# xuanjiangliu/robotic-discovery-platform

Measured on AMD Instinct MI355X. Metric: U-Net train imgs/sec at 256×256 (1/2/4/8 GPU); e2e frames/sec + p50 latency, higher is better.
Workload: dtype bf16; 1 GPU; model=UNet(3,1) bilinear decoder, 17.26M params, global_batch=64, per_gpu_batch=64, image_size=256, parallelism=dp1, impl=native, optimizer=Adam(lr=1e-4), loss=bce, sync_bn=False, hipgraph=False

## Files before the change

csrc/bindings.cpp:

```cpp
#include <torch/extension.h>
#include <c10/hip/HIPGuard.h>
#include <c10/hip/HIPStream.h>
#include <hip/hip_runtime.h>
#include <dlfcn.h>
#include <link.h>
#include <chrono>
#include <cmath>
#include <climits>
#include <cstdlib>
#include <cstring>
#include <functional>
#include <memory>
#include <vector>
#include <array>

#include "rdp_api.h"

namespace {

hipStream_t cur_stream() { return c10::hip::getCurrentHIPStream().stream(); }

void note_device(int& dev, const torch::Tensor& t) {
  if (!t.defined() || !t.is_cuda()) return;
  const int d = t.get_device();
// ... 698 lines not shown
  TORCH_CHECK(o.N == a.N && o.H == a.H && o.W == a.W && o.C == a.C, "bn bwd apply shape");
  TORCH_CHECK(RDP_PLAN(rdp_bn_relu_bwd_apply(d.ptr, d.pitch, a.ptr, a.pitch, coef.data_ptr<float>(), coef2.data_ptr<float>(),
                                    o.ptr, o.pitch, a.N * a.H * a.W, a.C, relu, st)) == 0, "bn bwd apply");
}

void maxpool2_fwd(torch::Tensor x, torch::Tensor out) {
  Act a = act(x, "x"), o = act(out, "out");
  TORCH_CHECK(o.N == a.N && o.H == a.H / 2 && o.W == a.W / 2 && o.C == a.C, "maxpool shape");
  TORCH_CHECK(RDP_PLAN(rdp_maxpool2_fwd(a.ptr, a.pitch, o.ptr, o.pitch, a.N, a.H, a.W, a.C, st)) == 0, "maxpool");
}

void maxpool2_bwd(torch::Tensor dp, torch::Tensor x, c10::optional<torch::Tensor> dskip, torch::Tensor dx) {
  Act p = act(dp, "dp"), a = act(x, "x"), o = act(dx, "dx"), s;
  if (dskip) { s = act(*dskip, "dskip"); TORCH_CHECK(s.N == a.N && s.H == a.H && s.W == a.W && s.C == a.C, "dskip shape"); }
  TORCH_CHECK(p.N == a.N && p.H == a.H / 2 && p.W == a.W / 2 && p.C == a.C, "maxpool bwd shape");
  TORCH_CHECK(o.N == a.N && o.H == a.H && o.W == a.W && o.C == a.C, "maxpool bwd dx shape");
  TORCH_CHECK(RDP_PLAN(rdp_maxpool2_bwd(p.ptr, p.pitch, a.ptr, a.pitch, dskip ? s.ptr : nullptr, dskip ? s.pitch : 0, o.ptr,
                               o.pitch, a.N, a.H, a.W, a.C, st)) == 0, "maxpool bwd");
}

void bn_relu_apply_pool(torch::Tensor y, c10::optional<torch::Tensor> out, torch::Tensor pool, torch::Tensor coef) {
  Act a = act(y, "y"), o, p = act(pool, "pool");
  if (out) {
    o = act(*out, "out");
    TORCH_CHECK(a.N == o.N && a.H == o.H && a.W == o.W && a.C == o.C, "bn_relu_apply_pool shape");
  }
  TORCH_CHECK(p.N == a.N && p.H == a.H / 2 && p.W == a.W / 2 && p.C == a.C, "bn_relu_apply_pool pool shape");
  check_f32(coef, "coef");
  TORCH_CHECK(coef.numel() >= 4 * a.C, "coef");
  TORCH_CHECK(RDP_PLAN(rdp_bn_relu_apply_pool(a.ptr, a.pitch, out ? o.ptr : nullptr, out ? o.pitch : 0, p.ptr, p.pitch, coef.data_ptr<float>(), a.N, a.H,
                                     a.W, a.C, st)) == 0, "bn_relu_apply_pool: channels must be 2^k in [8, 2048]");
}

int maxpool2_bwd_bn_reduce(torch::Tensor dp, torch::Tensor x, c10::optional<torch::Tensor> dskip, torch::Tensor dx,
                           torch::Tensor y, torch::Tensor coef, torch::Tensor partial) {
  Act p = act(dp, "dp"), a = act(x, "x"), o = act(dx, "dx"), yy = act(y, "y"), s;
  if (dskip) { s = act(*dskip, "dskip"); TORCH_CHECK(s.N == a.N && s.H == a.H && s.W == a.W && s.C == a.C, "dskip shape"); }
  TORCH_CHECK(p.N == a.N && p.H == a.H / 2 && p.W == a.W / 2 && p.C == a.C, "maxpool bwd shape");
  TORCH_CHECK(o.N == a.N && o.H == a.H && o.W == a.W && o.C == a.C, "maxpool bwd dx shape");
  TORCH_CHECK(yy.N == a.N && yy.H == a.H && yy.W == a.W && yy.C == a.C, "maxpool bwd y shape");
  check_f32(coef, "coef");
  check_f32(partial, "partial");
  TORCH_CHECK(coef.numel() >= 4 * a.C, "coef");
  const int maxb = partial.numel() / (2 * a.C);
  TORCH_CHECK(maxb >= 1, "partial too small");
  const int T = RDP_PLAN(rdp_maxpool2_bwd_bn_reduce(p.ptr, p.pitch, a.ptr, a.pitch, dskip ? s.ptr : nullptr, dskip ? s.pitch : 0,
                                           o.ptr, o.pitch, yy.ptr, yy.pitch, coef.data_ptr<float>(), a.N, a.H, a.W, a.C,
                                           partial.data_ptr<float>(), maxb, st));
  TORCH_CHECK(T > 0, "maxpool2_bwd_bn_reduce: channels must be 2^k in [8, 2048]");
  return T;
}

void upsample2_fwd(torch::Tensor x, torch::Tensor out, int oy, int ox, c10::optional<torch::Tensor> coef) {
  Act a = act(x, "x"), o = act(out, "out");
  TORCH_CHECK(o.N == a.N && o.C == a.C, "upsample shape");
  TORCH_CHECK(2 * a.H + oy <= o.H && 2 * a.W + ox <= o.W && oy >= 0 && ox >= 0, "upsample fwd placement");
  const float* cp = nullptr;
  if (coef && coef->defined()) {
    TORCH_CHECK(coef->is_cuda() && coef->scalar_type() == torch::kFloat32 && coef->numel() >= 4 * a.C, "coef [4C] f32");
    cp = coef->data_ptr<float>();
  }
  TORCH_CHECK(RDP_PLAN(rdp_upsample2_fwd(a.ptr, a.pitch, o.ptr, o.pitch, a.N, a.H, a.W, o.H, o.W, oy, ox, a.C, cp,
                                st)) == 0,
              "upsample fwd: channels must be 2^k in [8, 2048], pitches multiples of 8");
}

int upsample2_bwd(torch::Tensor dout, torch::Tensor dx, int oy, int ox, c10::optional<torch::Tensor> y,
                  c10::optional<torch::Tensor> coef, c10::optional<torch::Tensor> partial) {
  Act d = act(dout, "dout"), o = act(dx, "dx"), yy;
  TORCH_CHECK(o.N == d.N && o.C == d.C, "upsample bwd shape");
  TORCH_CHECK(2 * o.H + oy <= d.H && 2 * o.W + ox <= d.W && oy >= 0 && ox >= 0, "upsample bwd placement");
  const float* cf = nullptr;
  float* pp = nullptr;
  int maxb = 0;
  if (y) {
    TORCH_CHECK(coef && partial, "upsample2_bwd: y needs coef and partial");
    yy = act(*y, "y");
    TORCH_CHECK(yy.N == o.N && yy.H == o.H && yy.W == o.W && yy.C == o.C, "upsample bwd y shape");
    check_f32(*coef, "coef");
    check_f32(*partial, "partial");
    TORCH_CHECK(coef->numel() >= 4 * o.C, "coef");
    maxb = std::min<long>(partial->numel() / (2 * o.C), 4096);
    TORCH_CHECK(maxb >= 1, "partial too small");
// ... 1004 lines not shown
  m.def("plan_pause", &plan_pause);
  m.def("plan_resume", &plan_resume);
  m.def("plan_size", &plan_size);
  m.def("plan_free", &plan_free);
  m.def("conv_fwd", on_device(&conv_fwd), py::arg("x1"), py::arg("x2"), py::arg("w"), py::arg("taps"), py::arg("packed"),
        py::arg("y1"), py::arg("y2"), py::arg("stats"), py::arg("bm_pref"), py::arg("affine"), py::arg("relu"),
        py::arg("ws") = py::none(), py::arg("pool") = py::none(), py::arg("up") = py::none(),
        py::arg("up_oy") = 0, py::arg("up_ox") = 0, py::arg("wfrag") = py::none());
  m.def("conv_ws_elems", [](int N, int H, int W, int C1, int C2, int Cout, int taps, int packed, int bm_pref) {
    return rdp_conv_ws_elems(N, H, W, C1, C2, Cout, taps, packed, bm_pref);
  });
  m.def("conv_stats_rows", &conv_stats_rows);
  m.def("conv_wgrad", on_device(&conv_wgrad), py::arg("x1"), py::arg("x2"), py::arg("dy"), py::arg("taps"),
        py::arg("packed"), py::arg("cin_real"), py::arg("slab"), py::arg("out"), py::arg("accumulate"),
        py::arg("splits"), py::arg("variant"));
  m.def("conv_fwd_bnin", on_device(&conv_fwd_bnin), py::arg("x_pre"), py::arg("w"), py::arg("y"), py::arg("stats"),
        py::arg("in_coef"), py::arg("a_out") = py::none());
  m.def("wgrad_first_bn", on_device(&wgrad_first_bn));
  m.def("wgrad_slab_elems", &wgrad_slab_elems);
  m.def("wgrad_halo_slab_elems", &rdp_conv_wgrad_halo_slab_elems);
  m.def("bn_finalize", on_device(&bn_finalize));
  m.def("bn_eval_coef", on_device(&bn_eval_coef));
  m.def("bn_relu_apply", on_device(&bn_relu_apply));
  m.def("bn_relu_bwd_reduce", on_device(&bn_relu_bwd_reduce));
  m.def("conv_dgrad_bnred", on_device(&conv_dgrad_bnred));
  m.def("conv_dgrad_splitk_bnred", on_device(&conv_dgrad_splitk_bnred), py::arg("dy"), py::arg("w"), py::arg("dx"),
        py::arg("y_bn"), py::arg("coef"), py::arg("partial"), py::arg("ws") = py::none());
  m.def("bn_bwd_finalize", on_device(&bn_bwd_finalize));
  m.def("bn_relu_bwd_apply", on_device(&bn_relu_bwd_apply));
  m.def("maxpool2_fwd", on_device(&maxpool2_fwd));
  m.def("maxpool2_bwd", on_device(&maxpool2_bwd));
  m.def("bn_relu_apply_pool", on_device(&bn_relu_apply_pool));
  m.def("maxpool2_bwd_bn_reduce", on_device(&maxpool2_bwd_bn_reduce));
  m.def("upsample2_fwd", on_device(&upsample2_fwd), py::arg("x"), py::arg("out"), py::arg("oy"), py::arg("ox"),
        py::arg("coef") = py::none());
  m.def("upT_shuffle", on_device(&upT_shuffle));
  m.def("conv_upT_fwd", on_device(&conv_upT_fwd));
  m.def("conv_upT_dgrad", on_device(&conv_upT_dgrad));
  m.def("conv_wgrad_upT", on_device(&conv_wgrad_upT));
  m.def("upT_unshuffle", on_device(&upT_unshuffle));
  m.def("colsum_bf16", on_device(&colsum_bf16));
  m.def("upsample2_bwd", on_device(&upsample2_bwd), py::arg("dout"), py::arg("dx"), py::arg("oy"), py::arg("ox"),
        py::arg("y") = py::none(), py::arg("coef") = py::none(), py::arg("partial") = py::none());
  m.def("head_partial_blocks", &head_partial_blocks);
  m.def("head_fwd", on_device(&head_fwd), py::arg("a"), py::arg("w"), py::arg("b"), py::arg("target"), py::arg("logits"),
        py::arg("partial"), py::arg("sums"), py::arg("loss"), py::arg("dice_w"), py::arg("dice_eps"),
        py::arg("coef") = py::none(), py::arg("gpart") = py::none(), py::arg("bnpart") = py::none(),
        py::arg("gscale") = 1.0);
  m.def("head_grad_finalize", on_device(&head_grad_finalize));
  m.def("head_bwd", on_device(&head_bwd), py::arg("a"), py::arg("w"), py::arg("logits"), py::arg("target"), py::arg("sums"),
        py::arg("da"), py::arg("partial"), py::arg("gw"), py::arg("gb"), py::arg("dice_w"), py::arg("dice_eps"),
        py::arg("gscale"), py::arg("coef") = py::none(), py::arg("bnpart") = py::none());
  m.def("head_bn_bwd_apply", on_device(&head_bn_bwd_apply));
  m.def("head_mask", on_device(&head_mask));
  m.def("headk_partial_blocks", &headk_partial_blocks);
  m.def("headk_fwd", on_device(&headk_fwd), py::arg("a"), py::arg("w"), py::arg("b"), py::arg("labels"),
        py::arg("logits"), py::arg("partial"), py::arg("sums"), py::arg("loss"), py::arg("class_weights") = py::none(),
        py::arg("dice_w") = 0.0, py::arg("dice_eps") = 1.0);
  m.def("headk_bwd", on_device(&headk_bwd), py::arg("a"), py::arg("w"), py::arg("logits"), py::arg("labels"),
        py::arg("sums"), py::arg("da"), py::arg("partial"), py::arg("gw"), py::arg("gb"), py::arg("gscale") = 1.0,
        py::arg("class_weights") = py::none(), py::arg("dice_w") = 0.0, py::arg("dice_eps") = 1.0);
  m.def("headk_mask", on_device(&headk_mask), py::arg("a"), py::arg("w"), py::arg("b"), py::arg("cls"),
        py::arg("mask"));
  m.def("seg_confusion_blocks", &seg_confusion_blocks);
  m.def("seg_confusion_block_pixels", &seg_confusion_block_pixels);
  m.def("seg_confusion", on_device(&seg_confusion), py::arg("logits"), py::arg("target"), py::arg("K"),
// ... 63 lines not shown
```

csrc/pool_up.hip:

```cpp
#include "common.h"
#include "rdp_api.h"
#include <algorithm>

RDP_DEV void unpack8f(const uint4& v, float* f) {
  const uint32_t w[4] = {v.x, v.y, v.z, v.w};
#pragma unroll
  for (int k = 0; k < 4; ++k) {
    f[2 * k] = __uint_as_float(w[k] << 16);
    f[2 * k + 1] = __uint_as_float(w[k] & 0xffff0000u);
  }
}
RDP_DEV uint4 pack8f(const float* f) {
  uint4 v;
  v.x = pack2bf(f[0], f[1]);
  v.y = pack2bf(f[2], f[3]);
  v.z = pack2bf(f[4], f[5]);
  v.w = pack2bf(f[6], f[7]);
  return v;
}

__global__ void maxpool2_fwd_kernel(const u16* __restrict__ x, int xpitch, u16* __restrict__ out, int opitch, int N,
                                    int H, int W, int C) {
  const int Ho = H / 2, Wo = W / 2, CG = C >> 3;
  const long total = (long)N * Ho * Wo * CG;
// ... 103 lines not shown
    for (int q = 0; q < 4; ++q) {
      const int h = 2 * hc + (q >> 1), w = 2 * wc + (q & 1);
      ok[q] = h < H && w < W;
      px[q] = ((long)n * H + h) * W + w;
      if (ok[q]) v[q] = *(const uint4*)(y + px[q] * ypitch + c);
    }
    float av[4][8];
#pragma unroll
    for (int q = 0; q < 4; ++q) {
      if (!ok[q]) continue;
      float f[8];
      unpack8f(v[q], f);
#pragma unroll
      for (int k = 0; k < 8; ++k) f[k] = fmaxf(fmaf(f[k], ss[k], hh[k]), 0.f);
      const uint4 o = pack8f(f);
      if (a) *(uint4*)(a + px[q] * apitch + c) = o;
      unpack8f(o, av[q]);
    }
    if (hc < Ho && wc < Wo) {
      float o[8];
#pragma unroll
      for (int k = 0; k < 8; ++k) {
        float m = av[0][k];
#pragma unroll
        for (int q = 1; q < 4; ++q)
          if (av[q][k] > m || isnan(av[q][k])) m = av[q][k];
        o[k] = m;
      }
      *(uint4*)(pool + (((long)n * Ho + hc) * Wo + wc) * ppitch + c) = pack8f(o);
    }
  }
}

__global__ __launch_bounds__(256) void maxpool2_bwd_bn_reduce_kernel(
    const u16* __restrict__ dp, int dppitch, const u16* __restrict__ dskip,
    int dspitch, u16* __restrict__ dx, int dxpitch, const u16* __restrict__ y, int ypitch,
    const float* __restrict__ coef, int N, int H, int W, int C, float* __restrict__ partial) {
  extern __shared__ __attribute__((aligned(16))) float sred[];
  const int CG = C >> 3, RPB = 256 / CG;
  const int g = threadIdx.x & (CG - 1), r = threadIdx.x / CG;
  const int c = g * 8;
  float mean[8], inv[8], ss[8], hh[8];
  ld8f(coef + c, mean);
  ld8f(coef + C + c, inv);
  ld8f(coef + 2 * C + c, ss);
  ld8f(coef + 3 * C + c, hh);
  float sg[8], sgx[8];
#pragma unroll
  for (int k = 0; k < 8; ++k) { sg[k] = 0.f; sgx[k] = 0.f; }
  const int Ho = H / 2, Wo = W / 2, Hc = (H + 1) / 2, Wc = (W + 1) / 2;
  const int nwin = N * Hc * Wc;
  for (int wi = blockIdx.x * RPB + r; wi < nwin; wi += gridDim.x * RPB) {
    const int wc = wi % Wc, t = wi / Wc;
    const int hc = t % Hc, n = t / Hc;
    const bool pooled = hc < Ho && wc < Wo;
    bool ok[4];
    long px[4];
    uint4 vs[4], vy[4], vd;
#pragma unroll
    for (int q = 0; q < 4; ++q) {
      const int h = 2 * hc + (q >> 1), w = 2 * wc + (q & 1);
      ok[q] = h < H && w < W;
      px[q] = ((long)n * H + h) * W + w;
      if (ok[q]) {
        vy[q] = *(const uint4*)(y + px[q] * ypitch + c);
        vs[q] = dskip ? *(const uint4*)(dskip + px[q] * dspitch + c) : make_uint4(0, 0, 0, 0);
// ... 1 lines not shown
    }
    if (pooled) vd = *(const uint4*)(dp + (((long)n * Ho + hc) * Wo + wc) * dppitch + c);
    int idx[8];
    float d[8];
    if (pooled) {
      float v[4][8];
#pragma unroll
      for (int q = 0; q < 4; ++q) {
        float f[8];
        unpack8f(vy[q], f);
#pragma unroll
        for (int k = 0; k < 8; ++k) f[k] = fmaxf(fmaf(f[k], ss[k], hh[k]), 0.f);
        unpack8f(pack8f(f), v[q]);
      }
      unpack8f(vd, d);
#pragma unroll
      for (int k = 0; k < 8; ++k) {
        float m = v[0][k];
        int id = 0;
#pragma unroll
        for (int q = 1; q < 4; ++q)
          if (v[q][k] > m || isnan(v[q][k])) { m = v[q][k]; id = q; }
        idx[k] = id;
      }
    }
#pragma unroll
    for (int q = 0; q < 4; ++q) {
      if (!ok[q]) continue;
      float sk[8], o[8], fy[8];
      unpack8f(vs[q], sk);
#pragma unroll
      for (int k = 0; k < 8; ++k) o[k] = sk[k] + ((pooled && idx[k] == q) ? d[k] : 0.f);
      const uint4 ov = pack8f(o);
      *(uint4*)(dx + px[q] * dxpitch + c) = ov;
      unpack8f(ov, o);
      unpack8f(vy[q], fy);
#pragma unroll
      for (int k = 0; k < 8; ++k) {
        const float gg = fmaf(fy[k], ss[k], hh[k]) > 0.f ? o[k] : 0.f;
        sg[k] += gg;
        sgx[k] += gg * (fy[k] - mean[k]) * inv[k];
      }
    }
  }
#pragma unroll
  for (int k = 0; k < 8; ++k) {
    sred[(r * C + c + k) * 2] = sg[k];
    sred[(r * C + c + k) * 2 + 1] = sgx[k];
  }
  __syncthreads();
  for (int cc = threadIdx.x; cc < C; cc += 256) {
    float a0 = 0.f, a1 = 0.f;
    for (int q = 0; q < RPB; ++q) { a0 += sred[(q * C + cc) * 2]; a1 += sred[(q * C + cc) * 2 + 1]; }
    partial[(size_t)blockIdx.x * 2 * C + cc] = a0;
    partial[(size_t)blockIdx.x * 2 * C + C + cc] = a1;
  }
}

struct UpGeom {
  int N, hin, win, Hout, Wout, oy, ox, C;
  float rh, rw;
};

RDP_DEV void up_src(int u, int in, float r, int& i0, int& i1, float& l1) {
  const float s = r * (float)u;
  i0 = (int)s;
  i1 = i0 + (i0 < in - 1 ? 1 : 0);
  l1 = s - (float)i0;
}

RDP_DEV void bn_relu8(float* v, const float* sc, const float* sh) {
#pragma unroll
  for (int k = 0; k < 8; ++k) v[k] = bf2f(f2bf(fmaxf(fmaf(v[k], sc[k], sh[k]), 0.f)));
}

__global__ __launch_bounds__(256) void upsample2_fwd_taps_kernel(const u16* __restrict__ x, int xpitch,
                                                                 u16* __restrict__ out, int opitch, UpGeom g, int lcg,
                                                                 int nchunk, const float* __restrict__ coef) {
  const int CG = 1 << lcg;
  const int items = g.N * g.Hout * nchunk;
  for (int it = blockIdx.x; it < items; it += gridDim.x) {
    const int row = it / nchunk, q = it - row * nchunk;
    const int n = row / g.Hout, Y = row - n * g.Hout;
    const int t = q * 256 + threadIdx.x;
    const int X = t >> lcg, c = (t & (CG - 1)) * 8;
    if (X >= g.Wout) continue;
    const int uy = Y - g.oy, ux = X - g.ox;
    float o[8];
// ... 339 lines not shown

extern "C" {
int rdp_maxpool2_fwd(const void* x, int xpitch, void* out, int opitch, int N, int H, int W, int C, hipStream_t s) {
  if (C % 8 || xpitch % 8 || opitch % 8) return -1;
  hipLaunchKernelGGL(maxpool2_fwd_kernel, dim3(gridN((long)N * (H / 2) * (W / 2) * (C / 8))), dim3(256), 0, s,
                     (const u16*)x, xpitch, (u16*)out, opitch, N, H, W, C);
  return 0;
}
int rdp_maxpool2_bwd(const void* dp, int dppitch, const void* x, int xpitch, const void* dskip, int dspitch, void* dx,
                     int dxpitch, int N, int H, int W, int C, hipStream_t s) {
  if (C % 8) return -1;
  hipLaunchKernelGGL(maxpool2_bwd_kernel, dim3(gridN((long)N * ((H + 1) / 2) * ((W + 1) / 2) * (C / 8))), dim3(256),
                     0, s, (const u16*)dp, dppitch, (const u16*)x, xpitch, (const u16*)dskip, dspitch, (u16*)dx,
                     dxpitch, N, H, W, C);
  return 0;
}
static bool pow2c(int C) { return C >= 8 && C <= 2048 && (C & (C - 1)) == 0; }
int rdp_bn_relu_apply_pool(const void* y, int ypitch, void* a, int apitch, void* pool, int ppitch, const float* coef,
                           int N, int H, int W, int C, hipStream_t s) {
  if (!pow2c(C) || ypitch % 8 || apitch % 8 || ppitch % 8) return -1;
  const long rpb = 256 / (C / 8), nwin = (long)N * ((H + 1) / 2) * ((W + 1) / 2);
  const int grid = (int)std::max<long>(1, std::min<long>((nwin + rpb - 1) / rpb, 16384));
  hipLaunchKernelGGL(bn_relu_apply_pool_kernel, dim3(grid), dim3(256), 0, s, (const u16*)y, ypitch, (u16*)a, apitch,
                     (u16*)pool, ppitch, coef, N, H, W, C);
  return 0;
}
int rdp_maxpool2_bwd_bn_reduce(const void* dp, int dppitch, const void* x, int xpitch, const void* dskip, int dspitch,
                               void* dx, int dxpitch, const void* y, int ypitch, const float* coef, int N, int H, int W,
                               int C, float* partial, int max_blocks, hipStream_t s) {
  if (!pow2c(C) || dppitch % 8 || xpitch % 8 || dspitch % 8 || dxpitch % 8 || ypitch % 8) return -1;
  const long rpb = 256 / (C / 8), nwin = (long)N * ((H + 1) / 2) * ((W + 1) / 2);
  const int grid = (int)std::max<long>(1, std::min<long>((nwin + 4 * rpb - 1) / (4 * rpb), max_blocks));
  const size_t lds = (size_t)rpb * C * 2 * sizeof(float);
  hipLaunchKernelGGL(maxpool2_bwd_bn_reduce_kernel, dim3(grid), dim3(256), lds, s, (const u16*)dp, dppitch,
                     (const u16*)dskip, dspitch, (u16*)dx, dxpitch, (const u16*)y, ypitch, coef,
                     N, H, W, C, partial);
  return grid;
}
static int ilog2(int v) {
  int l = 0;
  while ((1 << l) < v) ++l;
  return l;
}
int rdp_upsample2_fwd(const void* x, int xpitch, void* out, int opitch, int N, int hin, int win, int Hout, int Wout,
                      int oy, int ox, int C, const float* coef, hipStream_t s) {
  if (!pow2c(C) || xpitch % 8 || opitch % 8) return -1;
  UpGeom g{N, hin, win, Hout, Wout, oy, ox, C, ac_scale(hin, 2 * hin), ac_scale(win, 2 * win)};
  const int lcg = ilog2(C / 8), nchunk = (int)(((long)Wout * (C / 8) + 255) / 256);
  int R = 8;
  while (R > 1 && (long)N * ((Hout + R - 1) / R) * nchunk < 4096) R >>= 1;
  const long items = (long)N * ((Hout + R - 1) / R) * nchunk;
  if (R == 1) {
    hipLaunchKernelGGL(upsample2_fwd_taps_kernel, dim3((int)std::min<long>(items, 8192)), dim3(256), 0, s,
                       (const u16*)x, xpitch, (u16*)out, opitch, g, lcg, nchunk, coef);
    return 0;
  }
  hipLaunchKernelGGL(upsample2_fwd_kernel, dim3((int)std::min<long>(items, 32768)), dim3(256), 0, s, (const u16*)x,
                     xpitch, (u16*)out, opitch, g, lcg, nchunk, R, coef);
  return 0;
}
int rdp_upsample2_bwd(const void* dout, int dpitch, void* dx, int xpitch, int N, int hin, int win, int Hout, int Wout,
                      int oy, int ox, int C, const void* y, int ypitch, const float* coef, float* partial,
                      int max_blocks, hipStream_t s) {
  if (!pow2c(C) || dpitch % 8 || xpitch % 8 || (y && ypitch % 8)) return -1;
  UpGeom g{N, hin, win, Hout, Wout, oy, ox, C, ac_scale(hin, 2 * hin), ac_scale(win, 2 * win)};
  const int lcg = ilog2(C / 8), nchunk = (int)(((long)win * (C / 8) + 255) / 256);
  int R = 4;
  while (R > 1 && (long)N * ((hin + R - 1) / R) * nchunk < 4096) R >>= 1;
  const long items = (long)N * ((hin + R - 1) / R) * nchunk;
  if (y) {
// ... 42 lines not shown
```

csrc/rdp_api.h:

```cpp
#pragma once
#include <hip/hip_runtime_api.h>

#include "rdp_host_api.h"

struct RdpConv {
  const void* x1 = nullptr;
  const void* x2 = nullptr;
  long xbytes1 = 0, xbytes2 = 0;
  int C1 = 0, C2 = 0, pitch1 = 0, pitch2 = 0;
  const void* w = nullptr;
  long wbytes = 0;
  int ldw = 0;
  void* y1 = nullptr;
  void* y2 = nullptr;
  long ybytes1 = 0, ybytes2 = 0;
  int Cy1 = 0, ypitch1 = 0, ypitch2 = 0;
  float* stats = nullptr;
  int N = 0, H = 0, W = 0, Cout = 0;
  const float* escale = nullptr;
  const float* eshift = nullptr;
  int erelu = 0;
};
struct RdpConvFuse {
  void* pool = nullptr;
// ... 142 lines not shown
int rdp_bn_eval_coef(int C, const float* gamma, const float* beta, const float* rmean, const float* rvar, float eps,
                     float* coef, hipStream_t s);
int rdp_bn_relu_apply(const void* y, int ypitch, void* out, int opitch, const float* coef, int M, int C, int relu,
                      hipStream_t s);
int rdp_bn_relu_bwd_reduce(const void* da, int dapitch, const void* y, int ypitch, const float* coef, int M, int C,
                           int relu, float* partial, int max_blocks, hipStream_t s);
int rdp_bn_bwd_finalize(const float* partial, int T, int C, long count, const float* gamma, const float* coef,
                        float* dgamma, float* dbeta, float* coef2, float* ws, hipStream_t s);
int rdp_bn_relu_bwd_apply(const void* da, int dapitch, const void* y, int ypitch, const float* coef,
                          const float* coef2, void* dy, int dypitch, int M, int C, int relu, hipStream_t s);

int rdp_adam(float* p, const void* g, int g_bf16, float* m, float* v, void* shadow, long n, float lr, float b1,
             float b2, float eps, float wd, float gscale, int* step, int inc, int max_blocks, hipStream_t s);
int rdp_adam_ctl(float* p, const void* g, int g_bf16, float* m, float* v, void* shadow, long n, float lr, float b1,
                 float b2, float eps, float wd, float gscale, int* step, const float* ctl, int inc, int max_blocks,
                 hipStream_t s);
int rdp_grad_sqnorm(const void* g, int g_bf16, long n, double* partial, int max_blocks, hipStream_t s);
int rdp_grad_sqnorm_blocks(long n);
int rdp_optim_ctl(const double* partial, int nblocks, double gscale, double clip, int sched, int W, int T, double r,
                  const int* step, float* ctl, hipStream_t s);
int rdp_cast_bf16(const float* p, void* out, long n, hipStream_t s);
int rdp_wprep(const float* master, void* out, const void* segs, int nseg, int* step, int tiles, int blocks,
              hipStream_t s);
int rdp_wseg_size();

int rdp_maxpool2_fwd(const void* x, int xpitch, void* out, int opitch, int N, int H, int W, int C, hipStream_t s);
int rdp_maxpool2_bwd(const void* dp, int dppitch, const void* x, int xpitch, const void* dskip, int dspitch,
                     void* dx, int dxpitch, int N, int H, int W, int C, hipStream_t s);
int rdp_bn_relu_apply_pool(const void* y, int ypitch, void* a, int apitch, void* pool, int ppitch,
                           const float* coef, int N, int H, int W, int C, hipStream_t s);
int rdp_maxpool2_bwd_bn_reduce(const void* dp, int dppitch, const void* x, int xpitch, const void* dskip,
                               int dspitch, void* dx, int dxpitch, const void* y, int ypitch, const float* coef,
                               int N, int H, int W, int C, float* partial, int max_blocks, hipStream_t s);
int rdp_upsample2_fwd(const void* x, int xpitch, void* out, int opitch, int N, int hin, int win, int Hout, int Wout,
                      int oy, int ox, int C, const float* coef, hipStream_t s);
int rdp_upsample2_bwd(const void* dout, int dpitch, void* dx, int xpitch, int N, int hin, int win, int Hout,
                      int Wout, int oy, int ox, int C, const void* y, int ypitch, const float* coef, float* partial,
                      int max_blocks, hipStream_t s);
int rdp_upT_shuffle(const void* yT, int ypitch, const float* bias, void* u, int upitch, int N, int h, int w, int H2,
                    int W2, int oy, int ox, int C, hipStream_t s);
int rdp_upT_unshuffle(const void* du, int dpitch, void* dyT, int ypitch, int N, int h, int w, int H2, int W2,
                      int oy, int ox, int C, hipStream_t s);
int rdp_colsum_bf16(const void* x, int pitch, long M, int K, int groups, float* partial, float* out, int accumulate,
                    hipStream_t s);

int rdp_seg_confusion_block_pixels();
int rdp_seg_confusion_blocks(long M);
int rdp_seg_confusion(const float* logits, const void* target, void* counts, long M, int K, float thr,
                      int max_blocks, hipStream_t s);

int rdp_preprocess(const void* bgr, int H, int W, const int* ystart, const int* ysize, const float* yw,
                   const int* xstart, const int* xsize, const float* xw, int OH, int OW, int rgb, void* out,
                   hipStream_t s);
int rdp_preprocess_batch(int n, const void* const* bgr, int H, int W, const int* ystart, const int* ysize,
                         const float* yw, const int* xstart, const int* xsize, const float* xw, int OH, int OW,
                         int rgb, void* const* out, hipStream_t s);
int rdp_mask_upsample(const void* m, int mh, int mw, void* out, int H, int W, unsigned* count, hipStream_t s);
int rdp_jpeg_gpu_batch(int n, const void* const* coefs, const int* const* geo, const int* const* qt,
                       void* const* planes, int H, int W, int max_blocks, void* const* rgb, hipStream_t s);
long rdp_jpeg_max_coefs(int H, int W);
long rdp_jpeg_plane_bytes(int H, int W);
int rdp_jpeg_gpu(const void* coefs, const int* geo, const int* qt, void* planes, int H, int W, int max_blocks,
                 void* rgb, hipStream_t s);
int rdp_h2d_copy(const void* src, void* dst, long bytes, hipStream_t s);
int rdp_h2d_copy_multi(const void* const* src, void* const* dst, const long* bytes, int n, hipStream_t s);

// ... 2 lines not shown
```

robotic_discovery_platform_amd/models/unet.py:

```python
from __future__ import annotations

import contextlib
import math
import os
from dataclasses import dataclass, field
from typing import Dict, List, Optional, Tuple

import torch
import torch.nn as nn

from .unet_ref import UNetRef, unet_widths

ALIGN = 64


@dataclass
class UpTSpec:
    name: str
    cin: int
    cout: int

    def param_names(self) -> List[str]:
        return [self.name + ".weight", self.name + ".bias"]

# ... 293 lines not shown
    def upT_dgrad_weight(self, us: UpTSpec) -> torch.Tensor:
        return self.store.flat_slice(us.name + ".weight", self.store.shadow).view(us.cin, 4 * us.cout)

    def forward(self, x: torch.Tensor) -> torch.Tensor:
        ex = self.executor(x.shape[0], x.shape[2], x.shape[3], training=False,
                           loss="ce" if self.n_classes > 1 else "bce")
        ex.set_input(x)
        ex.forward()
        return ex.logits_nchw()

    def executor(self, batch: int, h: int, w: int, training: bool = True, loss: str = "bce",
                 dice_weight: float = 1.0, class_weights=None) -> "UNetExecutor":
        if self.n_classes > 1 and loss not in ("ce", "ce_dice"):
            raise ValueError(f'a {self.n_classes}-class model trains with loss="ce" or "ce_dice", got {loss!r}')
        if self.n_classes == 1 and loss in ("ce", "ce_dice"):
            raise ValueError(f'loss={loss!r} needs n_classes > 1 (the one-class head takes "bce" / "bce_dice")')
        if self.n_classes == 1 and class_weights is not None:
            raise ValueError("class_weights need n_classes > 1")
        if loss == "ce_dice" and not 0.0 <= float(dice_weight) < float("inf"):
            raise ValueError(f"dice_weight must be finite and >= 0, got {dice_weight!r}")
        if class_weights is None:
            key = (batch, h, w, training, loss, dice_weight)
        else:
            from ..train.losses import check_class_weights
            class_weights = check_class_weights(class_weights, self.n_classes)
            key = (batch, h, w, training, loss, dice_weight, class_weights)
        cache = self.__dict__.setdefault("_executors", {})
        if key not in cache:
            cache[key] = UNetExecutor(self, batch, h, w, training, loss, dice_weight, class_weights)
        return cache[key]


class _Ablated:
    RET = {"bn_relu_bwd_reduce": 1, "conv_wgrad": 1, "wgrad_first_bn": 0, "conv_dgrad_bnred": 0}

    def __init__(self, C, names):
        self._C, self._names = C, frozenset(names)

    def __getattr__(self, n):
        if n in self._names and self._C.plan_recording():
            return lambda *a, **k: self.RET.get(n)
        return getattr(self._C, n)


_ABLATED = None



def rowband_frag_weights(w: torch.Tensor) -> torch.Tensor:
    co, k = w.shape
    return w.view(co // 16, 16, k // 32, 4, 8).permute(0, 2, 3, 1, 4).contiguous().view(co, k)

def _native():
    from ..ops import native
    global _ABLATED
    spec = os.environ.get("RDP_ABLATE", "")
    if not spec:
        return native()
    if _ABLATED is None:
        _ABLATED = _Ablated(native(), [n for n in spec.split(",") if n and n not in ("wgsum", "wgred")])
    return _ABLATED


@dataclass
class _Layer:
    spec: ConvSpec
    x1: torch.Tensor
    x2: Optional[torch.Tensor]
    y: torch.Tensor
    a: torch.Tensor
    coef: torch.Tensor
    coef2: torch.Tensor
    da: Optional[torch.Tensor] = None
    dy: Optional[torch.Tensor] = None
    dx1: Optional[torch.Tensor] = None
    dx1_owner: Optional["_Layer"] = None
    dx2: Optional[torch.Tensor] = None
    splits: int = 1
    bwd_rows: int = 0
    bnin: Optional["_Layer"] = None
    consumer_bnin: bool = False


_STREAM_OBSERVERS: List = []


_CONCURRENT_CACHE: Dict[tuple, bool] = {}


def _runs_concurrently(a: "torch.cuda.Stream", b: "torch.cuda.Stream") -> bool:
    key = (a.cuda_stream, b.cuda_stream)
    if key in _CONCURRENT_CACHE:
        return _CONCURRENT_CACHE[key]
    import time
    C = _native()
    torch.cuda.synchronize()
    best = 1e9
    for _ in range(2):
        t0 = time.perf_counter()
        with torch.cuda.stream(a):
            C.comm_emulate(300.0, 1)
        with torch.cuda.stream(b):
            C.comm_emulate(300.0, 1)
        torch.cuda.synchronize()
        best = min(best, time.perf_counter() - t0)
    ok = best < 450e-6
    _CONCURRENT_CACHE[key] = _CONCURRENT_CACHE[(key[1], key[0])] = ok
    return ok


def concurrent_stream(dev, others, tries: int = 8) -> "torch.cuda.Stream":
    others = [o for o in others if o is not None]
    if os.environ.get("RDP_STREAM_PROBE", "1") == "0" or torch.device(dev).type != "cuda":
        return torch.cuda.Stream(dev)
    s = None
    with torch.cuda.device(dev):
        for _ in range(tries):
            s = torch.cuda.Stream(dev)
            if all(_runs_concurrently(s, o) for o in others):
                return s
    return s


def _stream_wait(waiter: "torch.cuda.Stream", waitee: "torch.cuda.Stream"):
    _native().stream_wait(waiter.cuda_stream, waitee.cuda_stream)
    for o in _STREAM_OBSERVERS:
        o.wait(waiter, waitee)


class UNetExecutor:

    def __init__(self, model: UNetNative, N: int, H: int, W: int, training: bool, loss: str, dice_weight: float,
                 class_weights=None):
        self.m, self.N, self.H, self.W = model, N, H, W
        self.training = training
        self.loss_kind = loss
        self.dice_w = float(dice_weight) if loss in ("bce_dice", "ce_dice") else 0.0
        self.dice_eps = 1.0
        dev = model.store.device
        self.dev = dev
        self.class_weights = tuple(class_weights) if class_weights is not None else None
        self.class_w = (torch.tensor(self.class_weights, dtype=torch.float32, device=dev)
                        if class_weights is not None else None)
        self.K = model.n_classes
        self.fuse_head = training and self.K == 1
        self._mask_head_fused = False
        C = _native()
        D = model.depth
        bf = torch.bfloat16
        specs = model.specs
        enc = unet_widths(model.base_width, D, model.bilinear)
        sizes = [(H, W)]
        for _ in range(D):
            h, w = sizes[-1]
            sizes.append((h // 2, w // 2))
        self.sizes = sizes

        def t(h, w, c):
            return torch.zeros(N, h, w, c, dtype=bf, device=dev)

        self.x_in = t(H, W, 8)
        self.target = torch.zeros(N * H * W, dtype=torch.float32 if self.K == 1 else torch.uint8, device=dev)
        self.layers: List[_Layer] = []
# ... 322 lines not shown
                self._head_fwd_grads = True
            else:
                C.head_fwd(lb.y, head_w, head_b, self.target, self.logits, self.head_partial, self.loss_sums,
                           self.loss, self.dice_w, self.dice_eps, lb.coef)
        else:
            C.head_fwd(self.final, head_w, head_b, self.target, self.logits, self.head_partial, self.loss_sums,
                       self.loss, self.dice_w, self.dice_eps)

    def _conv_head_mask(self, C, L: _Layer, mask_head: tuple) -> bool:
        sp = L.spec
        if self.training or L.x2 is not None or sp.taps != 9 or sp.packed:
            return False
        if self.K > 1:
            if os.environ.get("RDP_SERVE_FUSED_HEADK", "1") == "0":
                return False
            if self.K == 5 and L.x1.shape[0] >= 4:
                return False
            hw, hb, cls, mask = mask_head
            return bool(C.conv_headk_mask(L.x1, self.m.fwd_weight(sp), L.coef, hw, hb, int(cls), mask))
        hw, hb, thr, mask = mask_head
        return bool(C.conv_head_mask(L.x1, self.m.fwd_weight(sp), L.coef, hw, hb, float(thr), mask))

    def logits_nchw(self) -> torch.Tensor:
        if self.K > 1:
            return self.logits.view(self.N, self.H, self.W, self.K).permute(0, 3, 1, 2)
        return self.logits.view(self.N, 1, self.H, self.W)

    def _bn_bwd(self, C, L: _Layer, head_gscale: Optional[float] = None, apply: bool = True):
        sp = L.spec
        st = self.m.store
        M = L.y.shape[0] * L.y.shape[1] * L.y.shape[2]
        T = L.bwd_rows if L.bwd_rows else C.bn_relu_bwd_reduce(L.da, L.y, L.coef, 1, self.bn_partial)
        L.bwd_rows = 0
        if self._sync_on:
            C.bn_bwd_finalize(self.bn_partial, T, M, st.view(sp.bn + ".weight"), L.coef,
                              st.view(sp.bn + ".weight", st.grad), st.view(sp.bn + ".bias", st.grad), L.coef2,
                              self.red_ws)
            T, M = self._sync_rows(self.bn_partial, T, sp.cout, (L.y.shape[1], L.y.shape[2]))
            C.bn_bwd_finalize(self.bn_partial, T, M, st.view(sp.bn + ".weight"), L.coef, None, None, L.coef2,
                              self.red_ws)
        else:
            C.bn_bwd_finalize(self.bn_partial, T, M, st.view(sp.bn + ".weight"), L.coef,
                              st.view(sp.bn + ".weight", st.grad), st.view(sp.bn + ".bias", st.grad), L.coef2,
                              self.red_ws)
        if not apply:
            return
        if head_gscale is not None:
            C.head_bn_bwd_apply(L.y, st.view("outc.conv.weight").reshape(-1), self.logits, self.target,
                                self.loss_sums, L.coef, L.coef2, L.dy, self.dice_w, self.dice_eps, head_gscale)
        else:
            C.bn_relu_bwd_apply(L.da, L.y, L.coef, L.coef2, L.dy, 1)

    def set_sync_bn(self, group=None, enabled: bool = True):
        import torch.distributed as dist
        if enabled and dist.is_available() and dist.is_initialized():
            if group is None:
                group = self.m.__dict__.get("_sync_bn_group")
                if group is None:
                    group = dist.new_group()
                    self.m.__dict__["_sync_bn_group"] = group
            self.sync_group, self.sync_world = group, dist.get_world_size(group)
            self.sync_comm = None
            if (group is self.m.__dict__.get("_sync_bn_group") and dist.get_backend(group) == "nccl"
                    and self.dev.type == "cuda" and os.environ.get("RDP_DDP_COMM", "native") == "native"):
                from ..parallel.ddp import emulate_spec, native_comm_group
                self.sync_comm = native_comm_group(self.dev, "syncbn")[1]
                self.sync_emulate = emulate_spec()
            self.sync_ws64 = torch.zeros(2 * max(L.spec.cout for L in self.layers), dtype=torch.float64,
                                         device=self.dev)
            shp = torch.tensor([self.N, self.H, self.W], dtype=torch.int64)
            if dist.get_backend(group) != "gloo":
                shp = shp.to(self.dev)
            shapes = [torch.zeros_like(shp) for _ in range(self.sync_world)]
            dist.all_gather(shapes, shp, group=group)
            self._sync_m = {}
            for lvl, (h, w) in enumerate(self.sizes):
                tot = 0
                for t in shapes:
                    n, hh, ww = (int(v) for v in t.tolist())
                    for _ in range(lvl):
                        hh, ww = hh // 2, ww // 2
                    tot += n * hh * ww
# ... 178 lines not shown
            ox = (du.shape[2] - 2 * low_layer.a.shape[2]) // 2
            if self.m.bilinear:
                low_layer.bwd_rows = C.upsample2_bwd(du, low_layer.da, oy, ox, low_layer.y, low_layer.coef,
                                                     self.bn_partial)
            else:
                us = self.m.up_specs[i - 1]
                dyT = self.dyTs[i - 1]
                bgrad = st.flat_slice(us.name + ".bias", st.grad)
                wgrad = st.flat_slice(us.name + ".weight", st.grad)
                ns = self.upT_splits[i - 1]
                exact = du.shape[1] == 2 * dyT.shape[1] and du.shape[2] == 2 * dyT.shape[2]
                if exact:
                    C.colsum_bf16(du, 1, self.colsum_ws, bgrad, 0)
                    self._on_wgrad_stream(lambda slab, du=du, xa=low_layer.a, ns=ns, g=wgrad:
                                          C.conv_wgrad_upT(du, xa, 0, 0, slab, g, 0, ns))
                    if C.conv_upT_dgrad(du, self.m.upT_dgrad_weight(us), low_layer.da, 0, 0) != 0:
                        C.upT_unshuffle(du, dyT, oy, ox)
                        C.conv_fwd(dyT, None, self.m.upT_dgrad_weight(us), 1, 0, low_layer.da, None, None, 0, None,
                                   0, self.kws)
                else:
                    C.upT_unshuffle(du, dyT, oy, ox)
                    C.colsum_bf16(dyT, 4, self.colsum_ws, bgrad, 0)
                    self._on_wgrad_stream(lambda slab, dyT=dyT, xa=low_layer.a, us=us, ns=ns, g=wgrad:
                                          C.conv_wgrad(dyT, None, xa, 1, 0, 4 * us.cout, slab, g, 0, ns, 0))
                    C.conv_fwd(dyT, None, self.m.upT_dgrad_weight(us), 1, 0, low_layer.da, None, None, 0, None, 0,
                               self.kws)
                if grad_hook is not None:
                    grad_hook(us, self.side if self.side is not None else torch.cuda.current_stream())
        for i in range(D, 0, -1):
            la, lb = self.down_layers[i]
            self._conv_bwd(C, lb, grad_hook)
            self._conv_bwd(C, la, grad_hook)
            prev = self.down_layers[i - 1][1]
            prev.bwd_rows = C.maxpool2_bwd_bn_reduce(self.dpools[i - 1], self.skips[i - 1], self.dskips[i - 1],
                                                     prev.da, prev.y, prev.coef, self.bn_partial)
        l0, l1 = self.down_layers[0]
        self._conv_bwd(C, l1, grad_hook)
        self._conv_bwd(C, l0, grad_hook)

    def backward_order(self) -> List:
        return backward_hook_order(self.m.specs, self.m.up_specs, self.m.depth)


def backward_hook_order(specs: List[ConvSpec], up_specs: List[UpTSpec], depth: int) -> List:
    D = depth
    enc = specs[: 2 * (D + 1)]
    dec = specs[2 * (D + 1):]
    out: List = [HEAD_SPEC]

    def conv(sp):
        out.extend([BNHook(sp), sp])

    for i in range(D, 0, -1):
        conv(dec[2 * (i - 1) + 1])
        conv(dec[2 * (i - 1)])
        if up_specs:
            out.append(up_specs[i - 1])
    for i in range(D, -1, -1):
        conv(enc[2 * i + 1])
        conv(enc[2 * i])
    return out


class NativeAdam:

    def __init__(self, model: UNetNative, lr: float = 1e-4, betas=(0.9, 0.999), eps: float = 1e-8,
                 weight_decay: float = 0.0, clip_grad_norm: float = 0.0, lr_schedule: str = "constant",
                 warmup_steps: int = 0, total_steps: Optional[int] = None, min_lr_ratio: float = 0.0):
# ... 119 lines not shown
```

Before: 3501 images/s.

## Skip storing pool-boundary activation gradient and recompute it in fused BN apply

For large encoder layers at the maxpool boundary, the fused maxpool-backward + BN-reduce kernel no longer writes the full activation gradient. A new fused kernel recomputes the maxpool backward from dpool/dskip during the BN-ReLU backward apply. This removes one full-size bf16 write and read in exchange for re-reading dp, dskip and y and redoing the argmax. A size-based heuristic selects two-pass mode, and reverses block traversal order at exactly 256MB, presumably for cache reuse with the preceding pass.

```diff
diff --git a/csrc/bindings.cpp b/csrc/bindings.cpp
--- a/csrc/bindings.cpp
+++ b/csrc/bindings.cpp
@@ -754,12 +754,12 @@
                                      a.W, a.C, st)) == 0, "bn_relu_apply_pool: channels must be 2^k in [8, 2048]");
 }
 
-int maxpool2_bwd_bn_reduce(torch::Tensor dp, torch::Tensor x, c10::optional<torch::Tensor> dskip, torch::Tensor dx,
-                           torch::Tensor y, torch::Tensor coef, torch::Tensor partial) {
-  Act p = act(dp, "dp"), a = act(x, "x"), o = act(dx, "dx"), yy = act(y, "y"), s;
+int maxpool2_bwd_bn_reduce(torch::Tensor dp, torch::Tensor x, c10::optional<torch::Tensor> dskip,
+                           c10::optional<torch::Tensor> dx, torch::Tensor y, torch::Tensor coef, torch::Tensor partial) {
+  Act p = act(dp, "dp"), a = act(x, "x"), o, yy = act(y, "y"), s;
   if (dskip) { s = act(*dskip, "dskip"); TORCH_CHECK(s.N == a.N && s.H == a.H && s.W == a.W && s.C == a.C, "dskip shape"); }
   TORCH_CHECK(p.N == a.N && p.H == a.H / 2 && p.W == a.W / 2 && p.C == a.C, "maxpool bwd shape");
-  TORCH_CHECK(o.N == a.N && o.H == a.H && o.W == a.W && o.C == a.C, "maxpool bwd dx shape");
+  if (dx) { o = act(*dx, "dx"); TORCH_CHECK(o.N == a.N && o.H == a.H && o.W == a.W && o.C == a.C, "maxpool bwd dx shape"); }
   TORCH_CHECK(yy.N == a.N && yy.H == a.H && yy.W == a.W && yy.C == a.C, "maxpool bwd y shape");
   check_f32(coef, "coef");
   check_f32(partial, "partial");
@@ -767,10 +767,25 @@
   const int maxb = partial.numel() / (2 * a.C);
   TORCH_CHECK(maxb >= 1, "partial too small");
   const int T = RDP_PLAN(rdp_maxpool2_bwd_bn_reduce(p.ptr, p.pitch, a.ptr, a.pitch, dskip ? s.ptr : nullptr, dskip ? s.pitch : 0,
-                                           o.ptr, o.pitch, yy.ptr, yy.pitch, coef.data_ptr<float>(), a.N, a.H, a.W, a.C,
-                                           partial.data_ptr<float>(), maxb, st));
+                                           dx ? o.ptr : nullptr, dx ? o.pitch : 0, yy.ptr, yy.pitch, coef.data_ptr<float>(),
+                                           a.N, a.H, a.W, a.C, partial.data_ptr<float>(), maxb, st));
   TORCH_CHECK(T > 0, "maxpool2_bwd_bn_reduce: channels must be 2^k in [8, 2048]");
   return T;
+}
+
+void maxpool2_bwd_bn_apply(torch::Tensor dp, c10::optional<torch::Tensor> dskip, torch::Tensor y, torch::Tensor coef,
+                           torch::Tensor coef2, torch::Tensor dy, int reverse) {
+  Act p = act(dp, "dp"), a = act(y, "y"), o = act(dy, "dy"), s;
+  if (dskip) { s = act(*dskip, "dskip"); TORCH_CHECK(s.N == a.N && s.H == a.H && s.W == a.W && s.C == a.C, "dskip shape"); }
+  TORCH_CHECK(p.N == a.N && p.H == a.H / 2 && p.W == a.W / 2 && p.C == a.C, "maxpool bwd shape");
+  TORCH_CHECK(o.N == a.N && o.H == a.H && o.W == a.W && o.C == a.C, "maxpool bwd dy shape");
+  check_f32(coef, "coef");
+  check_f32(coef2, "coef2");
+  TORCH_CHECK(coef.numel() >= 4 * a.C && coef2.numel() >= 3 * a.C, "coef [4C], coef2 [3C]");
+  TORCH_CHECK(RDP_PLAN(rdp_maxpool2_bwd_bn_apply(p.ptr, p.pitch, dskip ? s.ptr : nullptr, dskip ? s.pitch : 0, a.ptr, a.pitch,
+                                                 coef.data_ptr<float>(), coef2.data_ptr<float>(), o.ptr, o.pitch, a.N,
+                                                 a.H, a.W, a.C, reverse, st)) == 0,
+              "maxpool2_bwd_bn_apply: channels must be 2^k in [8, 2048], pitches multiples of 8");
 }
 
 void upsample2_fwd(torch::Tensor x, torch::Tensor out, int oy, int ox, c10::optional<torch::Tensor> coef) {
@@ -1841,6 +1856,12 @@
   m.def("maxpool2_bwd", on_device(&maxpool2_bwd));
   m.def("bn_relu_apply_pool", on_device(&bn_relu_apply_pool));
   m.def("maxpool2_bwd_bn_reduce", on_device(&maxpool2_bwd_bn_reduce));
+  m.def("maxpool2_bwd_bn_apply", on_device(&maxpool2_bwd_bn_apply), py::arg("dp"), py::arg("dskip"), py::arg("y"),
+        py::arg("coef"), py::arg("coef2"), py::arg("dy"), py::arg("reverse") = 0);
+  m.def("pool_bwd_two_pass", [](long M, int C) { return rdp_pool_bwd_two_pass(M, C) != 0; }, py::arg("M"), py::arg("C"),
+        "whether the native size table runs the pool boundary of an [M][C] layer without a stored activation gradient");
+  m.def("px_reverse", [](long M, int C) { return rdp_px_reverse(M, C); }, py::arg("M"), py::arg("C"),
+        "whether the native size table walks maxpool2_bwd_bn_apply over [M][C] back to front");
   m.def("upsample2_fwd", on_device(&upsample2_fwd), py::arg("x"), py::arg("out"), py::arg("oy"), py::arg("ox"),
         py::arg("coef") = py::none());
   m.def("upT_shuffle", on_device(&upT_shuffle));
diff --git a/csrc/pool_up.hip b/csrc/pool_up.hip
--- a/csrc/pool_up.hip
+++ b/csrc/pool_up.hip
@@ -159,6 +159,7 @@
   }
 }
 
+template <bool STORE>
 __global__ __launch_bounds__(256) void maxpool2_bwd_bn_reduce_kernel(
     const u16* __restrict__ dp, int dppitch, const u16* __restrict__ dskip,
     int dspitch, u16* __restrict__ dx, int dxpitch, const u16* __restrict__ y, int ypitch,
@@ -226,7 +227,7 @@
 #pragma unroll
       for (int k = 0; k < 8; ++k) o[k] = sk[k] + ((pooled && idx[k] == q) ? d[k] : 0.f);
       const uint4 ov = pack8f(o);
-      *(uint4*)(dx + px[q] * dxpitch + c) = ov;
+      if (STORE) *(uint4*)(dx + px[q] * dxpitch + c) = ov;
       unpack8f(ov, o);
       unpack8f(vy[q], fy);
 #pragma unroll
@@ -248,6 +249,86 @@
     for (int q = 0; q < RPB; ++q) { a0 += sred[(q * C + cc) * 2]; a1 += sred[(q * C + cc) * 2 + 1]; }
     partial[(size_t)blockIdx.x * 2 * C + cc] = a0;
     partial[(size_t)blockIdx.x * 2 * C + C + cc] = a1;
+  }
+}
+
+__global__ __launch_bounds__(256) void maxpool2_bwd_bn_apply_kernel(
+    const u16* __restrict__ dp, int dppitch, const u16* __restrict__ dskip, int dspitch,
+    const u16* __restrict__ y, int ypitch, const float* __restrict__ coef, const float* __restrict__ coef2,
+    u16* __restrict__ dy, int dypitch, int N, int H, int W, int C, int reverse) {
+  const int CG = C >> 3, RPB = 256 / CG;
+  const int g = threadIdx.x & (CG - 1), r = threadIdx.x / CG;
+  const int c = g * 8;
+  float ss[8], hh[8], A[8], B[8], K[8];
+  ld8f(coef + 2 * C + c, ss);
+  ld8f(coef + 3 * C + c, hh);
+  ld8f(coef2 + c, A);
+  ld8f(coef2 + C + c, B);
+  ld8f(coef2 + 2 * C + c, K);
+  const int Ho = H / 2, Wo = W / 2, Hc = (H + 1) / 2, Wc = (W + 1) / 2;
+  const int nwin = N * Hc * Wc;
+  const int blk = reverse ? (int)(gridDim.x - 1 - blockIdx.x) : (int)blockIdx.x;
+  const int stepw = gridDim.x * RPB;
+  const int nstep = nwin > blk * RPB ? (nwin - blk * RPB + stepw - 1) / stepw : 0;
+  for (int st = 0; st < nstep; ++st) {
+    const int wi = blk * RPB + (reverse ? nstep - 1 - st : st) * stepw + r;
+    if (wi >= nwin) continue;
+    const int wc = wi % Wc, t = wi / Wc;
+    const int hc = t % Hc, n = t / Hc;
+    const bool pooled = hc < Ho && wc < Wo;
+    bool ok[4];
+    long px[4];
+    uint4 vs[4], vy[4], vd;
+#pragma unroll
+    for (int q = 0; q < 4; ++q) {
+      const int h = 2 * hc + (q >> 1), w = 2 * wc + (q & 1);
+      ok[q] = h < H && w < W;
+      px[q] = ((long)n * H + h) * W + w;
+      if (ok[q]) {
+        vy[q] = *(const uint4*)(y + px[q] * ypitch + c);
+        vs[q] = dskip ? *(const uint4*)(dskip + px[q] * dspitch + c) : make_uint4(0, 0, 0, 0);
+      }
+    }
+    if (pooled) vd = *(const uint4*)(dp + (((long)n * Ho + hc) * Wo + wc) * dppitch + c);
+    int idx[8];
+    float d[8];
+    if (pooled) {
+      float v[4][8];
+#pragma unroll
+      for (int q = 0; q < 4; ++q) {
+        float f[8];
+        unpack8f(vy[q], f);
+#pragma unroll
+        for (int k = 0; k < 8; ++k) f[k] = fmaxf(fmaf(f[k], ss[k], hh[k]), 0.f);
+        unpack8f(pack8f(f), v[q]);
+      }
+      unpack8f(vd, d);
+#pragma unroll
+      for (int k = 0; k < 8; ++k) {
+        float m = v[0][k];
+        int id = 0;
+#pragma unroll
+        for (int q = 1; q < 4; ++q)
+          if (v[q][k] > m || isnan(v[q][k])) { m = v[q][k]; id = q; }
+        idx[k] = id;
+      }
+    }
+#pragma unroll
+    for (int q = 0; q < 4; ++q) {
+      if (!ok[q]) continue;
+      float sk[8], o[8], fy[8];
+      unpack8f(vs[q], sk);
+#pragma unroll
+      for (int k = 0; k < 8; ++k) o[k] = sk[k] + ((pooled && idx[k] == q) ? d[k] : 0.f);
+      unpack8f(pack8f(o), o);
+      unpack8f(vy[q], fy);
+#pragma unroll
+      for (int k = 0; k < 8; ++k) {
+        const float gg = fmaf(fy[k], ss[k], hh[k]) > 0.f ? o[k] : 0.f;
+        o[k] = fmaf(A[k], gg, fmaf(B[k], fy[k], K[k]));
+      }
+      *(uint4*)(dy + px[q] * dypitch + c) = pack8f(o);
+    }
   }
 }
 
@@ -653,10 +734,30 @@
   const long rpb = 256 / (C / 8), nwin = (long)N * ((H + 1) / 2) * ((W + 1) / 2);
   const int grid = (int)std::max<long>(1, std::min<long>((nwin + 4 * rpb - 1) / (4 * rpb), max_blocks));
   const size_t lds = (size_t)rpb * C * 2 * sizeof(float);
-  hipLaunchKernelGGL(maxpool2_bwd_bn_reduce_kernel, dim3(grid), dim3(256), lds, s, (const u16*)dp, dppitch,
-                     (const u16*)dskip, dspitch, (u16*)dx, dxpitch, (const u16*)y, ypitch, coef,
-                     N, H, W, C, partial);
+  if (dx)
+    hipLaunchKernelGGL(maxpool2_bwd_bn_reduce_kernel<true>, dim3(grid), dim3(256), lds, s, (const u16*)dp, dppitch,
+                       (const u16*)dskip, dspitch, (u16*)dx, dxpitch, (const u16*)y, ypitch, coef,
+                       N, H, W, C, partial);
+  else
+    hipLaunchKernelGGL(maxpool2_bwd_bn_reduce_kernel<false>, dim3(grid), dim3(256), lds, s, (const u16*)dp, dppitch,
+                       (const u16*)dskip, dspitch, (u16*)nullptr, 0, (const u16*)y, ypitch, coef,
+                       N, H, W, C, partial);
   return grid;
+}
+int rdp_pool_bwd_two_pass(long M, int C) { return M * C * 2 >= (256l << 20) ? 1 : 0; }
+int rdp_px_reverse(long M, int C) { return M * C * 2 == (256l << 20) ? 1 : 0; }
+int rdp_maxpool2_bwd_bn_apply(const void* dp, int dppitch, const void* dskip, int dspitch, const void* y, int ypitch,
+                              const float* coef, const float* coef2, void* dy, int dypitch, int N, int H, int W,
+                              int C, int reverse, hipStream_t s) {
+  if (!pow2c(C) || dppitch % 8 || dspitch % 8 || ypitch % 8 || dypitch % 8) return -1;
+  const long rpb = 256 / (C / 8), nwin = (long)N * ((H + 1) / 2) * ((W + 1) / 2);
+  if (nwin < 1 || (long)N * H * W > 0x7fffffffl) return -1;
+  const int grid = (int)std::max<long>(1, std::min<long>((nwin + rpb - 1) / rpb, 8192));
+  if (reverse < 0) reverse = rdp_px_reverse((long)N * H * W, C);
+  hipLaunchKernelGGL(maxpool2_bwd_bn_apply_kernel, dim3(grid), dim3(256), 0, s, (const u16*)dp, dppitch,
+                     (const u16*)dskip, dspitch, (const u16*)y, ypitch, coef, coef2, (u16*)dy, dypitch, N, H, W, C,
+                     reverse);
+  return 0;
 }
 static int ilog2(int v) {
   int l = 0;
diff --git a/csrc/rdp_api.h b/csrc/rdp_api.h
--- a/csrc/rdp_api.h
+++ b/csrc/rdp_api.h
@@ -198,6 +198,11 @@
 int rdp_maxpool2_bwd_bn_reduce(const void* dp, int dppitch, const void* x, int xpitch, const void* dskip,
                                int dspitch, void* dx, int dxpitch, const void* y, int ypitch, const float* coef,
                                int N, int H, int W, int C, float* partial, int max_blocks, hipStream_t s);
+int rdp_pool_bwd_two_pass(long M, int C);
+int rdp_px_reverse(long M, int C);
+int rdp_maxpool2_bwd_bn_apply(const void* dp, int dppitch, const void* dskip, int dspitch, const void* y, int ypitch,
+                              const float* coef, const float* coef2, void* dy, int dypitch, int N, int H, int W,
+                              int C, int reverse, hipStream_t s);
 int rdp_upsample2_fwd(const void* x, int xpitch, void* out, int opitch, int N, int hin, int win, int Hout, int Wout,
                       int oy, int ox, int C, const float* coef, hipStream_t s);
 int rdp_upsample2_bwd(const void* dout, int dpitch, void* dx, int xpitch, int N, int hin, int win, int Hout,
diff --git a/robotic_discovery_platform_amd/models/unet.py b/robotic_discovery_platform_amd/models/unet.py
--- a/robotic_discovery_platform_amd/models/unet.py
+++ b/robotic_discovery_platform_amd/models/unet.py
@@ -349,7 +349,8 @@
 
 
 class _Ablated:
-    RET = {"bn_relu_bwd_reduce": 1, "conv_wgrad": 1, "wgrad_first_bn": 0, "conv_dgrad_bnred": 0}
+    RET = {"bn_relu_bwd_reduce": 1, "conv_wgrad": 1, "wgrad_first_bn": 0, "conv_dgrad_bnred": 0,
+           "maxpool2_bwd_bn_reduce": 1, "maxpool2_bwd_bn_apply": None}
 
     def __init__(self, C, names):
         self._C, self._names = C, frozenset(names)
@@ -395,6 +396,7 @@
     dx2: Optional[torch.Tensor] = None
     splits: int = 1
     bwd_rows: int = 0
+    pool_bwd: Optional[tuple] = None
     bnin: Optional["_Layer"] = None
     consumer_bnin: bool = False
 
@@ -446,6 +448,8 @@
 
 
 class UNetExecutor:
+
+    pool_bwd_two_pass = None
 
     def __init__(self, model: UNetNative, N: int, H: int, W: int, training: bool, loss: str, dice_weight: float,
                  class_weights=None):
@@ -834,6 +838,7 @@
         M = L.y.shape[0] * L.y.shape[1] * L.y.shape[2]
         T = L.bwd_rows if L.bwd_rows else C.bn_relu_bwd_reduce(L.da, L.y, L.coef, 1, self.bn_partial)
         L.bwd_rows = 0
+        pool_bwd, L.pool_bwd = L.pool_bwd, None
         if self._sync_on:
             C.bn_bwd_finalize(self.bn_partial, T, M, st.view(sp.bn + ".weight"), L.coef,
                               st.view(sp.bn + ".weight", st.grad), st.view(sp.bn + ".bias", st.grad), L.coef2,
@@ -850,6 +855,8 @@
         if head_gscale is not None:
             C.head_bn_bwd_apply(L.y, st.view("outc.conv.weight").reshape(-1), self.logits, self.target,
                                 self.loss_sums, L.coef, L.coef2, L.dy, self.dice_w, self.dice_eps, head_gscale)
+        elif pool_bwd is not None:
+            C.maxpool2_bwd_bn_apply(pool_bwd[0], pool_bwd[1], L.y, L.coef, L.coef2, L.dy, -1)
         else:
             C.bn_relu_bwd_apply(L.da, L.y, L.coef, L.coef2, L.dy, 1)
 
@@ -1094,8 +1101,14 @@
             self._conv_bwd(C, lb, grad_hook)
             self._conv_bwd(C, la, grad_hook)
             prev = self.down_layers[i - 1][1]
+            two_pass = self.pool_bwd_two_pass
+            if two_pass is None:
+                n_, h_, w_, c_ = prev.y.shape
+                two_pass = C.pool_bwd_two_pass(n_ * h_ * w_, c_)
             prev.bwd_rows = C.maxpool2_bwd_bn_reduce(self.dpools[i - 1], self.skips[i - 1], self.dskips[i - 1],
-                                                     prev.da, prev.y, prev.coef, self.bn_partial)
+                                                     None if two_pass else prev.da, prev.y, prev.coef,
+                                                     self.bn_partial)
+            prev.pool_bwd = (self.dpools[i - 1], self.dskips[i - 1]) if two_pass else None
         l0, l1 = self.down_layers[0]
         self._conv_bwd(C, l1, grad_hook)
         self._conv_bwd(C, l0, grad_hook)
```

Result: no change. 3503 images/s, median of 6 (+0.0%).
